# UoB-HPC/neutral

Hardware: AMD Instinct MI355X
Metric: particle-steps/sec (higher is better)
Workload: dtype f64

## Files before the change

neutral_amd/csrc/neutral_tiled.hip:

```cpp
#include <cstdlib>
#include <cstring>
#include <type_traits>

#include "neutral_kernels.h"

#include "neutral_device.h"
#include "neutral_history.h"
#include "neutral_step_options.h"
#include "neutral_wave.h"

namespace neutral {

#ifndef NEUTRAL_STREAM_BLOCK
#define NEUTRAL_STREAM_BLOCK 1024
#endif
constexpr int kStreamBlock = NEUTRAL_STREAM_BLOCK;
constexpr int kChunkParticlesMax = 32768;
constexpr int kChunkParticlesMin = 1024;
constexpr int kStreamRefillMin = 56;
constexpr int kStreamRepeat = 64;
constexpr int kStreamRepeatOnePass = 128;
#ifdef NEUTRAL_NO_CARRIED_START
constexpr bool kCarriedStart = false;
#else
constexpr bool kCarriedStart = true;
#endif
constexpr int kSortBlock = 256;
constexpr int kSortItems = 16;
constexpr int kSortSegment = kSortBlock * kSortItems;
constexpr int kSortLdsBins = 8192;

enum Ctrl : int {
  kCtrlChunkHead = 0,
  kCtrlNumChunks = 1,
  kCtrlCollideCount = 2,
  kCtrlActive = 3,
  kCtrlMigrants = 4,
  kCtrlPassesUsed = 5,
  kCtrlWindowed = 6,
  kCtrlEmigrants = 7,
  kCtrlFirstInactive = 8,
  kCtrlLive = 9,
  kCtrlHops = 10,
  kCtrlOverflows = 11,
  kCtrlBatches = 12,
  kCtrlIdlePolls = 13,
};
constexpr unsigned kQueueEmpty = 0xFFFFFFFFu;
constexpr unsigned kQueueStayMin = 256;
constexpr unsigned kQueueBatchMin = 1024;
constexpr unsigned kQueueBatchMax = 4096;
constexpr unsigned kQueueIdlePollsMax = 1u << 20;
constexpr unsigned kUnwindowedBudget = 160;
constexpr double kMigrateMinFacets = 8.0;
constexpr int kMaxStreamPasses = 256;


constexpr unsigned kNoBucket = 0xFFFFFFFFu;

__device__ __forceinline__ unsigned sort_bucket(const TiledArgs& t, unsigned summary) {
  const int state = summary_state(summary);
  const unsigned cls = 3u - summary_reach(summary);
  const unsigned live = (t.reach_classes > 1)
                            ? summary_tile(summary) * (unsigned)t.reach_classes + cls
                            : summary_tile(summary);
  if (t.pass == 0) {
    return (state == kRecGone) ? kNoBucket : (state != kRecDead) ? live : (unsigned)t.nsort;
  }
  return (state == kRecMigrate) ? live : kNoBucket;
}

__device__ __forceinline__ const unsigned* sort_summaries(const TiledArgs& t) {
  return (t.pass == 0) ? t.info_in : t.info_out;
}

__device__ __forceinline__ bool pass_is_empty(const TiledArgs& t) {
  return t.pass > 0 && t.ctrl[kCtrlMigrants] == 0;
}
__device__ __forceinline__ bool step_is_broken(const SolveArgs& a) {
  return a.counters->aborted != 0u;
}

__global__ __launch_bounds__(kSortBlock) void tile_count_kernel(SolveArgs a, TiledArgs t) {
  extern __shared__ unsigned s_bins[];
  if (pass_is_empty(t) || (t.pass > 0 && step_is_broken(a))) {
    return;
  }
  const int nbins = t.nsort + 1;
  const bool in_lds = nbins <= kSortLdsBins;
  if (in_lds) {
    for (int b = threadIdx.x; b < nbins; b += kSortBlock) {
      s_bins[b] = 0;
    }
    __syncthreads();
  }
  const unsigned* info = sort_summaries(t);
  const long long base = (long long)blockIdx.x * kSortSegment;
#pragma unroll 4
  for (int k = 0; k < kSortItems; ++k) {
    const long long i = base + (long long)k * kSortBlock + threadIdx.x;
    const unsigned b = (i < t.sort_end) ? sort_bucket(t, info[i]) : kNoBucket;
    if (in_lds) {
      if (b != kNoBucket) {
        atomicAdd(&s_bins[b], 1u);
      }
    } else {
      const bool is_dead = (b == (unsigned)t.nsort);
      const unsigned long long m_dead = __ballot(is_dead);
      if (b != kNoBucket && !is_dead) {
        atomicAdd(&t.tile_count[b], 1u);
      }
      if (m_dead != 0 && (threadIdx.x & 63) == (unsigned)__ffsll((long long)m_dead) - 1u) {
        atomicAdd(&t.tile_count[t.nsort], (unsigned)__popcll(m_dead));
      }
    }
  }
  if (in_lds) {
    __syncthreads();
    for (int b = threadIdx.x; b < nbins; b += kSortBlock) {
      const unsigned c = s_bins[b];
      if (c) {
        atomicAdd(&t.tile_count[b], c);
      }
    }
  }
}

__global__ __launch_bounds__(1024) void tile_scan_kernel(TiledArgs t) {
  __shared__ unsigned s_part[1024];
  const int tid = threadIdx.x;
  const int n = t.nsort + 2;
  const int per = (n + 1023) / 1024;
  const int lo = (tid * per < n) ? tid * per : n;
  const int hi = (lo + per < n) ? lo + per : n;
  unsigned sum = 0;
  for (int i = lo; i < hi; ++i) {
    sum += (i <= t.nsort) ? t.tile_count[i] : 0u;
  }
  s_part[tid] = sum;
  __syncthreads();
  for (int off = 1; off < 1024; off <<= 1) {
    const unsigned c0 = (tid >= off) ? s_part[tid - off] : 0;
    __syncthreads();
    s_part[tid] += c0;
    __syncthreads();
  }
  if (tid == 0) {
    t.ctrl[kCtrlWindowed] = 0;
  }
  unsigned run = s_part[tid] - sum;
  for (int i = lo; i < hi; ++i) {
    const unsigned c = (i <= t.nsort) ? t.tile_count[i] : 0u;
    t.tile_offset[i] = run;
    t.tile_cursor[i] = run;
    if (i <= t.nsort) {
      t.tile_count[i] = 0;
    }
    run += c;
  }
}

__device__ __forceinline__ void draw_for_slot(const SolveArgs& a, const TiledArgs& t, long long slot) {
  t.carried_in[slot].minus_log_rn0 = draw_first_flight(a.pid_base + (uint64_t)t.id_in[slot], a.master_key);
}

__global__ __launch_bounds__(kSortBlock) void tile_scatter_kernel(SolveArgs a, TiledArgs t) {
  extern __shared__ unsigned s_bins[];
  if (pass_is_empty(t) || (t.pass > 0 && step_is_broken(a))) {
    return;
  }
  const bool draws = t.pass == 0 && t.carried != 0;
  const int nbins = t.nsort + 1;
  const bool in_lds = nbins <= kSortLdsBins;
  unsigned* s_rank = s_bins;
  unsigned* s_base = s_bins + nbins;
  const unsigned* info = sort_summaries(t);
  const long long base = (long long)blockIdx.x * kSortSegment;
  unsigned bucket[kSortItems];
#pragma unroll
  for (int k = 0; k < kSortItems; ++k) {
    const long long i = base + (long long)k * kSortBlock + threadIdx.x;
    bucket[k] = (i < t.sort_end) ? sort_bucket(t, info[i]) : kNoBucket;
  }
  if (!in_lds) {
#pragma unroll
    for (int k = 0; k < kSortItems; ++k) {
      const bool is_dead = (bucket[k] == (unsigned)t.nsort);
      const unsigned long long m_dead = __ballot(is_dead);
      unsigned dead_base = 0;
      if (m_dead != 0) {
        const unsigned leader = (unsigned)__ffsll((long long)m_dead) - 1u;
        if ((threadIdx.x & 63) == leader) {
          dead_base = atomicAdd(&t.tile_cursor[t.nsort], (unsigned)__popcll(m_dead));
        }
        dead_base = __shfl(dead_base, (int)leader, 64);
      }
      if (bucket[k] != kNoBucket) {
        const unsigned pos = is_dead ? dead_base + (unsigned)lane_rank(m_dead)
                                     : atomicAdd(&t.tile_cursor[bucket[k]], 1u);
        t.order[pos] = (unsigned)(base + (long long)k * kSortBlock + threadIdx.x);
        if (draws && !is_dead) {
          draw_for_slot(a, t, base + (long long)k * kSortBlock + threadIdx.x);
        }
      }
    }
    return;
  }
  for (int b = threadIdx.x; b < nbins; b += kSortBlock) {
    s_rank[b] = 0;
  }
  __syncthreads();
#pragma unroll
  for (int k = 0; k < kSortItems; ++k) {
    if (bucket[k] != kNoBucket) {
      atomicAdd(&s_rank[bucket[k]], 1u);
    }
  }
  __syncthreads();
  for (int b = threadIdx.x; b < nbins; b += kSortBlock) {
    const unsigned c = s_rank[b];
    if (c) {
      s_base[b] = atomicAdd(&t.tile_cursor[b], c);
      s_rank[b] = 0;
    }
  }
  __syncthreads();
#pragma unroll
  for (int k = 0; k < kSortItems; ++k) {
    if (bucket[k] != kNoBucket) {
      const unsigned pos = s_base[bucket[k]] + atomicAdd(&s_rank[bucket[k]], 1u);
      t.order[pos] = (unsigned)(base + (long long)k * kSortBlock + threadIdx.x);
    }
  }
  if (draws) {
#pragma unroll 1
    for (int k = 0; k < kSortItems; ++k) {
      if (bucket[k] != kNoBucket && bucket[k] != (unsigned)t.nsort) {
        draw_for_slot(a, t, base + (long long)k * kSortBlock + threadIdx.x);
      }
    }
  }
}

__global__ __launch_bounds__(kSortBlock) void copy_inactive_kernel(SolveArgs a, TiledArgs t) {
  if (a.abort_flag && *a.abort_flag) {
    return;
  }
  const unsigned first_inactive = t.tile_offset[t.nsort];
  const unsigned ncarried = (unsigned)t.sort_end - first_inactive;
  const unsigned total = ncarried + (unsigned)(t.mirror_end - t.sort_end);
  for (unsigned u = blockIdx.x * kSortBlock + threadIdx.x; u < total; u += gridDim.x * kSortBlock) {
  if (u < ncarried) {
    const unsigned j = first_inactive + u;
    const unsigned src = t.order[j];
    const ParticleRec r = t.rec_in[src];
    t.rec_out[j] = r;
    t.info_out[j] = t.info_in[src];
    if (a.decomposed) {
      t.id_out[j] = t.id_in[src];
    } else {
      t.slot_of_id[r.id] = j;
    }
  } else {
    const unsigned m = (unsigned)t.sort_end + (u - ncarried);
    if (m < (unsigned)t.mirror_end) {
      t.rec_out[m] = t.rec_in[m];
      t.info_out[m] = t.info_in[m];
    }
  }
  }
}

__global__ __launch_bounds__(kSortBlock) void collect_suspended_kernel(SolveArgs a, TiledArgs t,
                                                                       const unsigned* info) {
  __shared__ unsigned s_count[kSortItems][kSortBlock / 64];
  __shared__ unsigned s_base;
  if (step_is_broken(a)) {
    return;
  }
  const long long base = (long long)blockIdx.x * kSortSegment;
  const int wave = threadIdx.x >> 6;
  unsigned mine = 0;
#pragma unroll
  for (int k = 0; k < kSortItems; ++k) {
    const long long i = base + (long long)k * kSortBlock + threadIdx.x;
    const bool susp = i < t.sort_end && summary_state(info[i]) == kRecCollide;
    const unsigned long long m = __ballot(susp);
    mine |= susp ? (1u << k) : 0u;
    if ((threadIdx.x & 63) == 0) {
      s_count[k][wave] = (unsigned)__popcll(m);
    }
  }
  __syncthreads();
  if (threadIdx.x == 0) {
    unsigned total = 0;
    for (int k = 0; k < kSortItems; ++k) {
      for (int w = 0; w < kSortBlock / 64; ++w) {
        const unsigned c = s_count[k][w];
        s_count[k][w] = total;
        total += c;
      }
    }
    s_base = total ? atomicAdd(&t.ctrl[kCtrlCollideCount], total) : 0u;
  }
  __syncthreads();
  if (mine) {
#pragma unroll
    for (int k = 0; k < kSortItems; ++k) {
      const bool susp = ((mine >> k) & 1u) != 0;
      const unsigned long long m = __ballot(susp);
      if (susp) {
        const unsigned slot = (unsigned)(base + (long long)k * kSortBlock + threadIdx.x);
        t.collide_queue[s_base + s_count[k][wave] + (unsigned)lane_rank(m)] = slot;
        if (t.mark_suspended) {
          const unsigned id = t.rec_out[slot].id;
          atomicOr(&t.susp_ids[id >> 5], 1u << (id & 31u));
        }
      }
    }
  }
}

__global__ __launch_bounds__(kSortBlock) void import_records_kernel(ParticleView p, ParticleRec* rec,
                                                                    unsigned* info,
                                                                    unsigned* slot_of_id,
                                                                    unsigned* ids, int tiles_x,
                                                                    int tile_shift, int x_off,
                                                                    int y_off, int n) {
  const int i = blockIdx.x * kSortBlock + threadIdx.x;
  if (i < n) {
    ParticleRec r;
    r.x = p.x[i];
    r.y = p.y[i];
    r.omega_x = p.omega_x[i];
    r.omega_y = p.omega_y[i];
    r.energy = p.energy[i];
    r.weight = p.weight[i];
    r.dt_to_census = p.dt_to_census[i];
    r.mfp_to_collision = p.mfp_to_collision[i];
    r.cellx = p.cellx[i];
    r.celly = p.celly[i];
    r.id = (unsigned)i;
    r.dead = p.dead[i];
    rec[i] = r;
    slot_of_id[i] = (unsigned)i;
    ids[i] = (unsigned)i;
    info[i] = slot_summary(r.dead ? kRecDead : kRecIdle, r.cellx - x_off, r.celly - y_off, tiles_x,
                           tile_shift);
  }
}

__global__ __launch_bounds__(kSortBlock) void refresh_micro_kernel(SolveArgs a, TiledArgs t) {
  const long long i = (long long)blockIdx.x * kSortBlock + threadIdx.x;
  if (i >= t.sort_end) {
    return;
  }
  const int state = summary_state(t.info_in[i]);
  if (state == kRecDead || state == kRecGone) {
    return;
  }
  const double energy = t.rec_in[i].energy;
  const int ind = cs_bracket(a.scatter_keys, a.scatter_n, energy);
  t.carried_in[i].micro = a.checked ? cs_interpolate<true>(a.scatter_keys, a.scatter_values, ind, energy)
                            : cs_interpolate<false>(a.scatter_keys, a.scatter_values, ind, energy);
}

__global__ __launch_bounds__(kSortBlock) void export_records_kernel(const ParticleRec* rec,
                                                                    const unsigned* slot_of_id,
                                                                    ParticleView p, int n,
                                                                    const int* abort_flag,
                                                                    const unsigned* first_inactive,
                                                                    unsigned final_from,
                                                                    const unsigned* skip_ids,
                                                                    int partial_ok) {
  if (abort_flag && *abort_flag) {
    return;
  }
  for (long long kk = (long long)blockIdx.x * kSortBlock + threadIdx.x; kk < n; kk += (long long)gridDim.x * kSortBlock) {
    const int k = (int)kk;
    if (skip_ids && ((skip_ids[k >> 5] >> (k & 31)) & 1u)) {
      continue;
    }
    const unsigned slot = slot_of_id[k];
    if (slot >= (first_inactive ? *first_inactive : final_from)) {
      continue;
    }
    const rec_quad* const q = (const rec_quad*)__builtin_assume_aligned(&rec[slot], 16);
    ParticleRec r;
    rec_quad* const rq = (rec_quad*)&r;
    rq[0] = q[0];
    rq[1] = q[1];
    rq[2] = q[2];
    __builtin_nontemporal_store(r.x, &p.x[k]);
    __builtin_nontemporal_store(r.y, &p.y[k]);
    __builtin_nontemporal_store(r.dt_to_census, &p.dt_to_census[k]);
    __builtin_nontemporal_store(r.mfp_to_collision, &p.mfp_to_collision[k]);
    __builtin_nontemporal_store(r.cellx, &p.cellx[k]);
    __builtin_nontemporal_store(r.celly, &p.celly[k]);
    if (!partial_ok || (r.dead & kRecChanged)) {
      rq[3] = q[3];
      rq[4] = q[4];
      __builtin_nontemporal_store(r.omega_x, &p.omega_x[k]);
      __builtin_nontemporal_store(r.omega_y, &p.omega_y[k]);
      __builtin_nontemporal_store(r.energy, &p.energy[k]);
      __builtin_nontemporal_store(r.weight, &p.weight[k]);
      __builtin_nontemporal_store((record_state(r.dead) == kRecDead) ? 1 : 0, &p.dead[k]);
    }
  }
}

__global__ __launch_bounds__(1024) void tile_chunks_kernel(TiledArgs t) {
  __shared__ unsigned s_chunks[1024];
  constexpr int kStagedOffsets = 8192;
  __shared__ unsigned s_offset[kStagedOffsets + 2];
  const int tid = threadIdx.x;
  const bool staged = t.nsort + 1 <= kStagedOffsets;
  if (staged) {
    for (int i = tid; i <= t.nsort + 1; i += 1024) {
      s_offset[i] = t.tile_offset[i];
    }
    __syncthreads();
  }
  const unsigned* offset = staged ? s_offset : t.tile_offset;
  const unsigned nactive = offset[t.nsort];
  const int classes = t.reach_classes;
  long long per = (t.ntiles + 1023) / 1024;
  if (nactive > 0) {
    const long long per_sparse =
        ((long long)t.chunk_particles * (long long)t.ntiles + nactive - 1) / (long long)nactive;
    per = (per_sparse > per) ? per_sparse : per;
    constexpr long long kSweepTilesMax = 32;
    const long long floor_per = (t.ntiles + 1023) / 1024;
    const long long cap = (floor_per > kSweepTilesMax) ? floor_per : kSweepTilesMax;
    per = (per > cap) ? cap : per;
  }
  per = (per > t.ntiles) ? t.ntiles : per;
  const long long lo_ll = (long long)tid * per;
  const int lo = (lo_ll < t.ntiles) ? (int)lo_ll : t.ntiles;
  const int hi = (lo_ll + per < t.ntiles) ? (int)(lo_ll + per) : t.ntiles;
  const unsigned cp = (unsigned)t.chunk_particles;

  unsigned nch = 0;
  unsigned chunk = 0;
  unsigned nwindowed = 0;
  for (int sweep = 0; sweep < 2; ++sweep) {
    unsigned run_begin = 0, run_end = 0;
    auto emit = [&](unsigned begin, unsigned end, unsigned tile, unsigned windowed) {
      if (end <= begin) {
        return;
      }
      const unsigned parts = (end - begin + cp - 1) / cp;
      const unsigned size = (end - begin + parts - 1) / parts;
      for (unsigned b = begin; b < end; b += size) {
        const unsigned e = (b + size < end) ? b + size : end;
        if (sweep == 0) {
          nch++;
        } else {
          const unsigned w = (windowed && (e - b) >= (unsigned)t.window_min_particles) ? 1u : 0u;
          if (chunk < (unsigned)t.max_chunks) {
            t.chunks[chunk] = make_uint4(b, e, tile, w);
          }
          nwindowed += w;
          chunk++;
        }
      }
    };
    for (int i = lo; i < hi; ++i) {
      const unsigned begin = offset[i * classes];
      const unsigned end = offset[(i + 1) * classes];
      if (end - begin >= (unsigned)t.window_min_particles) {
        emit(run_begin, run_end, 0u, 0u);
        run_begin = run_end = end;
        emit(begin, end, (unsigned)i, 1u);
      } else {
        if (run_end == run_begin) {
          run_begin = begin;
        }
        run_end = end;
      }
    }
    emit(run_begin, run_end, 0u, 0u);
    if (sweep == 0) {
      s_chunks[tid] = nch;
      __syncthreads();
      for (int off = 1; off < 1024; off <<= 1) {
        const unsigned c0 = (tid >= off) ? s_chunks[tid - off] : 0;
        __syncthreads();
        s_chunks[tid] += c0;
        __syncthreads();
      }
      chunk = s_chunks[tid] - nch;
    }
  }
  if (nwindowed) {
    atomicAdd(&t.ctrl[kCtrlWindowed], nwindowed);
  }
  if (tid == 1023) {
    t.ctrl[kCtrlNumChunks] = s_chunks[1023];
    t.ctrl[kCtrlActive] = nactive;
    t.ctrl[kCtrlLive] = nactive;
    t.ctrl[kCtrlChunkHead] = 0;
    t.ctrl[kCtrlCollideCount] = 0;
    t.ctrl[kCtrlMigrants] = 0;
    if (t.pass == 0) {
      t.ctrl[kCtrlPassesUsed] = 1;
      t.ctrl[kCtrlEmigrants] = 0;
      t.ctrl[kCtrlFirstInactive] = offset[t.nsort];
    } else if (nactive > 0) {
      t.ctrl[kCtrlPassesUsed] = (unsigned)t.pass + 1u;
    }
  }
}

__global__ __launch_bounds__(kSortBlock) void tile_uniform_kernel(SolveArgs a, TiledArgs t, int window_cells) {
  __shared__ int s_differs;
  if (threadIdx.x == 0) {
    s_differs = 0;
  }
  __syncthreads();
  const int tile = (int)blockIdx.x;
  const int margin = (window_cells - (1 << t.tile_shift)) >> 1;
  int x0 = ((tile % t.tiles_x) << t.tile_shift) - margin - 1;
  int y0 = ((tile / t.tiles_x) << t.tile_shift) - margin - 1;
  int x1 = x0 + window_cells + 2;
  int y1 = y0 + window_cells + 2;
  x0 = (x0 < 0) ? 0 : x0;
  y0 = (y0 < 0) ? 0 : y0;
  x1 = (x1 > a.nx) ? a.nx : x1;
  y1 = (y1 > a.ny) ? a.ny : y1;
  const int w = x1 - x0;
  const int n = w * (y1 - y0);
  const long long first = __double_as_longlong(a.density[(size_t)y0 * a.nx + x0]);
  bool differs = false;
  for (int i = threadIdx.x; i < n; i += kSortBlock) {
    const int y = y0 + i / w;
    const int x = x0 + i % w;
    differs |= (__double_as_longlong(a.density[(size_t)y * a.nx + x]) != first);
  }
  if (__ballot(differs) != 0 && (threadIdx.x & 63) == 0) {
    s_differs = 1;
  }
  __syncthreads();
  if (threadIdx.x == 0) {
    t.tile_uniform[tile] = s_differs ? 0 : 1;
  }
}

__global__ __launch_bounds__(1024) void edges_check_kernel(SolveArgs a, TiledArgs t) {
  __shared__ int s_differs;
  if (threadIdx.x == 0) {
    s_differs = 0;
  }
  __syncthreads();
  bool differs = !(a.edge_dx > 0.0) || !(a.edge_dy > 0.0);
  for (int i = threadIdx.x; i <= a.nx; i += 1024) {
    differs |= __double_as_longlong(edge_from_formula(a.edge_dx, i + a.x_off)) !=
               __double_as_longlong(a.edgex[i + a.pad]);
  }
  for (int i = threadIdx.x; i <= a.ny; i += 1024) {
    differs |= __double_as_longlong(edge_from_formula(a.edge_dy, i + a.y_off)) !=
               __double_as_longlong(a.edgey[i + a.pad]);
  }
  if (__ballot(differs) != 0 && (threadIdx.x & 63) == 0) {
    s_differs = 1;
  }
  __syncthreads();
  if (threadIdx.x == 0) {
    *t.edges_computed = s_differs ? 0 : 1;
  }
}


__global__ __launch_bounds__(kSortBlock) void queue_reset_kernel(TiledArgs t) {
  const int tile = (int)blockIdx.x;
  unsigned used = t.queue_tail[tile];
  used = (used > t.queue_capacity) ? t.queue_capacity : used;
  unsigned* log = t.queue_entries + (size_t)tile * t.queue_capacity;
  for (unsigned i = threadIdx.x; i < used; i += kSortBlock) {
    log[i] = kQueueEmpty;
  }
  __syncthreads();
  if (threadIdx.x == 0) {
    t.queue_tail[tile] = 0u;
    t.queue_head[tile] = 0u;
  }
}

template <int kW>
__device__ __forceinline__ void flush_window(const SolveArgs& a, double* window, double* mesh,
                                             int ox, int oy) {
  constexpr int kS = kW + kWindowRowPad;
  for (int i = threadIdx.x; i < kW * kW; i += kStreamBlock) {
    const int at = (i / kW) * kS + (i % kW);
    const double v = window[at];
    window[at] = 0.0;
    if (v != 0.0) {
      const int gx = ox + (i % kW);
      const int gy = oy + (i / kW);
      if (gx >= 0 && gx < a.nx && gy >= 0 && gy < a.ny) {
        unsafeAtomicAdd(&mesh[gy * a.nx + gx], v);
      }
    }
  }
}

template <bool kSameTables, bool kWithIndex = true>
__host__ __device__ __forceinline__ size_t stream_lds_payload_bytes(const SolveArgs& a, int window_cells) {
  size_t lds = sizeof(double) * (size_t)window_cells;
  if (kWithIndex && a.scatter_index) {
    lds += sizeof(unsigned short) * (size_t)(a.scatter_index_n + 1);
  }
  if (kWithIndex && !kSameTables && a.absorb_index) {
    lds += sizeof(unsigned short) * (size_t)(a.absorb_index_n + 1);
  }
  return (lds + 15) & ~(size_t)15;
}
#ifdef NEUTRAL_PHASE_CLOCK
constexpr size_t kStreamLdsControlBytes = 64 + 16 * 9 * 8;
#else
// ... 1047 lines not shown
```

Baseline: 152.1 billion.

## Split first-flight draws between count and scatter; vectorize suspended-collection loads

Moves first-flight random draws for the first half of each thread's sort items from the scatter kernel into the count kernel, spreading the RNG work across two passes. Rewrites collect_suspended_kernel to load summaries as uint4 runs per thread and to replace the single-thread serial offset scan with a wave-level shuffle scan. The new layout changes the queue order within a block, and the count kernel gains extra register pressure and scattered stores to carried_in.

```diff
diff --git a/neutral_amd/csrc/neutral_tiled.hip b/neutral_amd/csrc/neutral_tiled.hip
--- a/neutral_amd/csrc/neutral_tiled.hip
+++ b/neutral_amd/csrc/neutral_tiled.hip
@@ -81,6 +81,11 @@
   return a.counters->aborted != 0u;
 }
 
+constexpr int kSortDrawsInCount = kSortItems / 2;
+__device__ __forceinline__ void draw_for_slot(const SolveArgs& a, const TiledArgs& t, long long slot) {
+  t.carried_in[slot].minus_log_rn0 = draw_first_flight(a.pid_base + (uint64_t)t.id_in[slot], a.master_key);
+}
+
 __global__ __launch_bounds__(kSortBlock) void tile_count_kernel(SolveArgs a, TiledArgs t) {
   extern __shared__ unsigned s_bins[];
   if (pass_is_empty(t) || (t.pass > 0 && step_is_broken(a))) {
@@ -96,10 +101,13 @@
   }
   const unsigned* info = sort_summaries(t);
   const long long base = (long long)blockIdx.x * kSortSegment;
+  const bool draws = kSortDrawsInCount > 0 && t.pass == 0 && t.carried != 0;
+  unsigned to_draw = 0;
 #pragma unroll 4
   for (int k = 0; k < kSortItems; ++k) {
     const long long i = base + (long long)k * kSortBlock + threadIdx.x;
     const unsigned b = (i < t.sort_end) ? sort_bucket(t, info[i]) : kNoBucket;
+    to_draw |= (k < kSortDrawsInCount && b != kNoBucket && b != (unsigned)t.nsort) ? (1u << k) : 0u;
     if (in_lds) {
       if (b != kNoBucket) {
         atomicAdd(&s_bins[b], 1u);
@@ -121,6 +129,14 @@
       const unsigned c = s_bins[b];
       if (c) {
         atomicAdd(&t.tile_count[b], c);
+      }
+    }
+  }
+  if (draws) {
+#pragma unroll 1
+    for (int k = 0; k < kSortDrawsInCount; ++k) {
+      if ((to_draw >> k) & 1u) {
+        draw_for_slot(a, t, base + (long long)k * kSortBlock + threadIdx.x);
       }
     }
   }
@@ -158,10 +174,6 @@
     }
     run += c;
   }
-}
-
-__device__ __forceinline__ void draw_for_slot(const SolveArgs& a, const TiledArgs& t, long long slot) {
-  t.carried_in[slot].minus_log_rn0 = draw_first_flight(a.pid_base + (uint64_t)t.id_in[slot], a.master_key);
 }
 
 __global__ __launch_bounds__(kSortBlock) void tile_scatter_kernel(SolveArgs a, TiledArgs t) {
@@ -199,7 +211,7 @@
         const unsigned pos = is_dead ? dead_base + (unsigned)lane_rank(m_dead)
                                      : atomicAdd(&t.tile_cursor[bucket[k]], 1u);
         t.order[pos] = (unsigned)(base + (long long)k * kSortBlock + threadIdx.x);
-        if (draws && !is_dead) {
+        if (draws && !is_dead && k >= kSortDrawsInCount) {
           draw_for_slot(a, t, base + (long long)k * kSortBlock + threadIdx.x);
         }
       }
@@ -234,7 +246,7 @@
   }
   if (draws) {
 #pragma unroll 1
-    for (int k = 0; k < kSortItems; ++k) {
+    for (int k = kSortDrawsInCount; k < kSortItems; ++k) {
       if (bucket[k] != kNoBucket && bucket[k] != (unsigned)t.nsort) {
         draw_for_slot(a, t, base + (long long)k * kSortBlock + threadIdx.x);
       }
@@ -271,50 +283,98 @@
   }
 }
 
+constexpr int kSortRun = 4;
+constexpr int kSortRuns = kSortItems / kSortRun;
+static_assert(kSortRun == 4, "a run is one uint4");
+constexpr unsigned kSummaryBeyond = (unsigned)kRecGone << (32 - kRecStateBits);
+
+__device__ __forceinline__ long long sort_item(long long base, int k) {
+  return base + (long long)((k / kSortRun) * (kSortBlock * kSortRun) + (int)threadIdx.x * kSortRun +
+                            (k % kSortRun));
+}
+
+__device__ __forceinline__ void load_summaries(const unsigned* info, long long base, long long end,
+                                               unsigned (&s)[kSortItems]) {
+#pragma unroll
+  for (int c = 0; c < kSortRuns; ++c) {
+    const long long i0 = sort_item(base, c * kSortRun);
+    if (i0 + kSortRun <= end) {
+      const uint4 v = *reinterpret_cast<const uint4*>(info + i0);
+      s[c * kSortRun + 0] = v.x;
+      s[c * kSortRun + 1] = v.y;
+      s[c * kSortRun + 2] = v.z;
+      s[c * kSortRun + 3] = v.w;
+    } else {
+#pragma unroll
+      for (int j = 0; j < kSortRun; ++j) {
+        s[c * kSortRun + j] = (i0 + j < end) ? info[i0 + j] : kSummaryBeyond;
+      }
+    }
+  }
+}
+
 __global__ __launch_bounds__(kSortBlock) void collect_suspended_kernel(SolveArgs a, TiledArgs t,
                                                                        const unsigned* info) {
-  __shared__ unsigned s_count[kSortItems][kSortBlock / 64];
+  constexpr int kWaves = kSortBlock / 64;
+  __shared__ unsigned s_count[kSortRuns * kWaves];
   __shared__ unsigned s_base;
   if (step_is_broken(a)) {
     return;
   }
   const long long base = (long long)blockIdx.x * kSortSegment;
   const int wave = threadIdx.x >> 6;
+  unsigned summary[kSortItems];
+  load_summaries(info, base, t.sort_end, summary);
   unsigned mine = 0;
+  unsigned before[kSortRuns];
 #pragma unroll
-  for (int k = 0; k < kSortItems; ++k) {
-    const long long i = base + (long long)k * kSortBlock + threadIdx.x;
-    const bool susp = i < t.sort_end && summary_state(info[i]) == kRecCollide;
-    const unsigned long long m = __ballot(susp);
-    mine |= susp ? (1u << k) : 0u;
+  for (int c = 0; c < kSortRuns; ++c) {
+    unsigned in_wave = 0;
+    before[c] = 0;
+#pragma unroll
+    for (int j = 0; j < kSortRun; ++j) {
+      const bool susp = summary_state(summary[c * kSortRun + j]) == kRecCollide;
+      const unsigned long long m = __ballot(susp);
+      mine |= susp ? (1u << (c * kSortRun + j)) : 0u;
+      before[c] += (unsigned)lane_rank(m);
+      in_wave += (unsigned)__popcll(m);
+    }
     if ((threadIdx.x & 63) == 0) {
-      s_count[k][wave] = (unsigned)__popcll(m);
+      s_count[c * kWaves + wave] = in_wave;
     }
   }
   __syncthreads();
-  if (threadIdx.x == 0) {
-    unsigned total = 0;
-    for (int k = 0; k < kSortItems; ++k) {
-      for (int w = 0; w < kSortBlock / 64; ++w) {
-        const unsigned c = s_count[k][w];
-        s_count[k][w] = total;
-        total += c;
-      }
-    }
-    s_base = total ? atomicAdd(&t.ctrl[kCtrlCollideCount], total) : 0u;
+  if (threadIdx.x < 64) {
+    static_assert(kSortRuns * kWaves <= 64, "one lane per (run, wave)");
+    const unsigned c0 = (threadIdx.x < kSortRuns * kWaves) ? s_count[threadIdx.x] : 0u;
+    unsigned incl = c0;
+#pragma unroll
+    for (int off = 1; off < kSortRuns * kWaves; off <<= 1) {
+      const unsigned up = (unsigned)__shfl_up((int)incl, off, 64);
+      incl += (threadIdx.x >= (unsigned)off) ? up : 0u;
+    }
+    if (threadIdx.x < kSortRuns * kWaves) {
+      s_count[threadIdx.x] = incl - c0;
+    }
+    if (threadIdx.x == kSortRuns * kWaves - 1) {
+      s_base = incl ? atomicAdd(&t.ctrl[kCtrlCollideCount], incl) : 0u;
+    }
   }
   __syncthreads();
   if (mine) {
+    const unsigned seg_base = s_base;
 #pragma unroll
-    for (int k = 0; k < kSortItems; ++k) {
-      const bool susp = ((mine >> k) & 1u) != 0;
-      const unsigned long long m = __ballot(susp);
-      if (susp) {
-        const unsigned slot = (unsigned)(base + (long long)k * kSortBlock + threadIdx.x);
-        t.collide_queue[s_base + s_count[k][wave] + (unsigned)lane_rank(m)] = slot;
-        if (t.mark_suspended) {
-          const unsigned id = t.rec_out[slot].id;
-          atomicOr(&t.susp_ids[id >> 5], 1u << (id & 31u));
+    for (int c = 0; c < kSortRuns; ++c) {
+      unsigned at = seg_base + s_count[c * kWaves + wave] + before[c];
+#pragma unroll
+      for (int j = 0; j < kSortRun; ++j) {
+        if ((mine >> (c * kSortRun + j)) & 1u) {
+          const unsigned slot = (unsigned)sort_item(base, c * kSortRun + j);
+          t.collide_queue[at++] = slot;
+          if (t.mark_suspended) {
+            const unsigned id = t.rec_out[slot].id;
+            atomicOr(&t.susp_ids[id >> 5], 1u << (id & 31u));
+          }
         }
       }
     }
```

After: 149.2 billion, median of 2. About the same (-1.9%).
